# wzx99/DCFP

Hardware: AMD Instinct MI355X
Metric: training images/sec at 1024x2048 DeepLabv3-R101 (higher is better)
Workload: dtype f32; 1 GPU; DeepLabv3-resnet101+ASPP os8, 4x3x1024x2048 per GPU, CE+0.4*deepsup CE (fused upsample), 3x3 stride-1 convs with >= 256 channels as fp32 Winograd F(2x2,3x3) (fwd / dgrad / wgrad), all other convs direct implicit GEMM, EIC step, SGD m0.9 wd5e-4; global_batch=4, parallelism=dp1

## Files before the change

dcfp_amd/_lib.py:

```python
import ctypes as C
import os
import subprocess
import threading

_HERE = os.path.dirname(os.path.abspath(__file__))
LIB_PATH = os.environ.get("DCFP_LIB") or os.path.join(_HERE, "libdcfp_hip.so")
CSRC = os.path.join(_HERE, "csrc")

_lib = None
_lock = threading.Lock()


class ConvDesc(C.Structure):
    _fields_ = [(n, C.c_int32) for n in
                ("N", "Cin", "H", "W", "Cout", "KH", "KW", "stride", "pad", "dil", "Hout", "Wout",
                 "x_pitch", "dy_pitch")]


class ConvF16Desc(C.Structure):
    _fields_ = [(n, C.c_int32) for n in
                ("N", "H", "W", "Cin8", "x_pitch", "Cout", "K", "stride", "pad", "dil", "Hout", "Wout",
                 "y_pitch", "y_off", "res_pitch", "res_off", "relu")]


# ... 43 lines not shown

class VoteMap(C.Structure):
    _fields_ = [("logits", C.c_void_p)] + [(n, C.c_int32) for n in ("h", "w", "hs", "ws", "flip")] + \
               [("weight", C.c_float)]


AUG_SATURATION, AUG_HUE = 1, 2
SGD_CHUNK = 16384
CONV_FWD, CONV_DGRAD, CONV_WGRAD = 0, 1, 2
E_BADDESC, E_UNSUPPORTED, E_WORKSPACE = -1, -2, -3

_P, _I, _L, _F, _Z = C.c_void_p, C.c_int, C.c_int64, C.c_float, C.c_size_t
_D = C.POINTER(ConvDesc)
_R = C.POINTER(BnRunning)
_H = C.POINTER(ConvF16Desc)

SIGNATURES = {
    "dcfp_abi_version": (_I, []),
    "dcfp_conv2d_workspace_bytes": (_Z, [_D, _I]),
    "dcfp_conv2d_wp_layout": (_I, [_D, _I, C.POINTER(WpEntry)]),
    "dcfp_conv2d_permute_weights_multi_f32": (_I, [_P, _I, _L, _P]),
    "dcfp_conv2d_pitch_supported": (_I, [_D]),
    "dcfp_conv2d_kernel_name": (_I, [_D, _I, C.c_char_p, _I]),
    "dcfp_conv2d_executed_fraction": (C.c_double, [_D, _I]),
    "dcfp_conv2d_workspace_is_scratch": (_I, [_D, _I]),
    "dcfp_conv2d_dgrad_fanin_supported": (_I, [_D]),
    "dcfp_conv2d_dgrad_fanin_f32_nchw": (_I, [_D, _P, _L, _P, _P, _P, _P, _P, _Z, _I, _P]),
    "dcfp_conv2d_dgrad_fanin_red_slots": (_L, [_D]),
    "dcfp_conv2d_dgrad_fanin_red_f32_nchw": (_I, [_D, _P, _L, _P, _P, _P, _P, _P, _P, _P, _P, _P, _Z, _I, _P]),
    "dcfp_bn_bwd_sums_from_partials_f32": (_I, [_P, _L, _I, _P, _F, _P, _P, _P, _P, _P]),
    "dcfp_conv2d_xform_bytes": (_Z, [_D]),
    "dcfp_conv2d_fwd_keep_f32_nchw": (_I, [_D, _P, _P, _P, _L, _P, _Z, _P, _P, _Z, _P]),
    "dcfp_conv2d_wgrad_kept_f32_nchw": (_I, [_D, _P, _L, _P, _Z, _P, _P, _Z, _P]),
    "dcfp_conv2d_fwd_f32_nchw": (_I, [_D, _P, _P, _P, _P, _L, _P, _Z, _I, _P]),
    "dcfp_conv2d_fwd_fused_f32_nchw": (_I, [_D, _P, _P, _P, _P, _P, _I, _P, _P, _Z, _I, _P]),
    "dcfp_conv2d_dgrad_f32_nchw": (_I, [_D, _P, _L, _P, _P, _I, _P, _Z, _I, _P]),
    "dcfp_conv2d_wgrad_f32_nchw": (_I, [_D, _P, _L, _P, _P, _P, _P, _Z, _P]),
    "dcfp_bn_workspace_bytes": (_Z, [_I, _I, _I]),
    "dcfp_bn_stats_f32": (_I, [_P, _L, _I, _I, _I, _P, _P, _R, _P, _Z, _P]),
    "dcfp_bn_apply_f32": (_I, [_P, _P, _P, _P, _P, _F, _P, _I, _P, _L, _I, _I, _I, _I, _I, _P]),
    "dcfp_bn_bwd_reduce_f32": (_I, [_P, _L, _P, _P, _L, _P, _P, _P, _P, _F, _I, _I, _I, _I, _P, _P, _P, _P,
                                    _P, _Z, _P]),
    "dcfp_bn_update_running_f32": (_I, [_P, _P, _I, _F, _F, _P, _P, _P, _P]),
    "dcfp_syncbn_combine_f32": (_I, [_P, _I, _I, _P, _P, _P, _R, _P]),
    "dcfp_syncbn_p2p_mailbox_bytes": (_Z, [_I, _I]),
    "dcfp_p2p_alloc": (_I, [_Z, _I, C.POINTER(C.c_void_p)]),
    "dcfp_p2p_free": (_I, [_P]),
    "dcfp_p2p_export": (_I, [_P, _P]),
    "dcfp_p2p_import": (_I, [_P, C.POINTER(C.c_void_p)]),
    "dcfp_p2p_unmap": (_I, [_P]),
    "dcfp_syncbn_p2p_exchange_f32": (_I, [C.POINTER(C.c_void_p), _I, _I, C.c_uint32, _I, _P, _I, _I, _P, _R,
                                          C.c_uint32, _P, _P]),
    "dcfp_bn_apply_relu_mask_f32": (_I, [_P, _P, _P, _P, _P, _F, _P, _P, _P, _I, _I, _I, _P]),
    "dcfp_conv2d_fwd_stat_slots": (_L, [_D, _P, _L]),
    "dcfp_conv2d_fwd_stats_f32_nchw": (_I, [_D, _P, _P, _P, _L, _P, _P, _Z, _I, _P]),
    "dcfp_bn_stats_from_partials_f32": (_I, [_P, _L, _I, _I, _P, _P, _R, _P]),
    "dcfp_bn_bwd_apply_f32": (_I, [_P, _L, _P, _P, _L, _P, _P, _P, _P, _F, _P, _P, _F, _P, _I, _P, _P,
                                   _I, _I, _I, _I, _I, _P]),
    "dcfp_bn_bwd_fused_sync_bytes": (_Z, [_I, _I, _I]),
    "dcfp_bn_bwd_fused_f32": (_I, [_P, _L, _P, _P, _L, _P, _P, _P, _P, _F, _F, _I, _P, _P, _I, _I, _I, _I, _I,
                                   _P, _P, _P, _P, _P, _Z, C.c_uint32, C.c_uint32, _P, _P]),
    "dcfp_maxpool3x3s2_fwd_f32": (_I, [_P, _P, _P, _I, _I, _I, _I, _I, _I, _P]),
    "dcfp_maxpool3x3s2_bwd_f32": (_I, [_P, _P, _P, _I, _I, _I, _I, _I, _I, _P]),
    "dcfp_rowsum_f32": (_I, [_P, _L, _P, _F, _I, _I, _I, _P]),
    "dcfp_broadcast_hw_f32": (_I, [_P, _F, _P, _L, _I, _I, _I, _I, _P]),
    "dcfp_add_f32": (_I, [_P, _P, _P, _L, _P]),
# ... 89 lines not shown
```

dcfp_amd/csrc/conv_igemm2.hip:

```cpp
#include "igemm2_common.h"
#include <queue>
#include <vector>
#include <stdio.h>
#include <stdlib.h>

namespace {

__device__ __forceinline__ int wp_row(int m, int perm8) {
    if (!perm8) return m;
    const int j = m & 255;
    return (m & ~255) + 32 * (j & 7) + (j >> 3);
}

__global__ void __launch_bounds__(256)
permute_weights_kernel(const float* __restrict__ w, float* __restrict__ wp, int T, int Ck, int CkP,
                       int M, int Mpad, int sAm, int sAc, int perm8) {
    const long long total = (long long)T * CkP * Mpad;
    for (long long i = (long long)blockIdx.x * 256 + threadIdx.x; i < total;
         i += (long long)gridDim.x * 256) {
        const int m = wp_row((int)(i % Mpad), perm8);
        const long long r = i / Mpad;
        const int c = (int)(r % CkP);
        const int t = (int)(r / CkP);
        float v = 0.f;
        if (m < M && c < Ck) v = w[(long long)m * sAm + (long long)c * sAc + t];
        wp[i] = v;
    }
}

constexpr int kWpBlockElems = DCFP_WP_BLOCK_ELEMS;
__global__ void __launch_bounds__(256)
permute_weights_multi_kernel(const DcfpWpEntry* __restrict__ table, int n) {
    const long long blk = blockIdx.x;
    int lo = 0, hi = n - 1;
    while (lo < hi) {
        const int mid = (lo + hi + 1) >> 1;
        if (table[mid].first_block <= blk) lo = mid; else hi = mid - 1;
    }
    const DcfpWpEntry e = table[lo];
    const long long base = (blk - e.first_block) * kWpBlockElems;
    if (e.perm8 >= 2) {
        const long long pairs = (long long)e.CkP * e.Mpad;
#pragma unroll 1
        for (int u = 0; u < kWpBlockElems / 256; ++u) {
            const long long i = base + u * 256 + threadIdx.x;
            if (i >= pairs) return;
            wino_filter2_pair(e.w, e.sAm, e.sAc, e.perm8 == 3, e.M, e.Ck, e.Mpad, i, e.wp);
        }
        return;
    }
    const long long total = (long long)e.T * e.CkP * e.Mpad;
#pragma unroll
    for (int u = 0; u < kWpBlockElems / 256; ++u) {
        const long long i = base + u * 256 + threadIdx.x;
        if (i >= total) return;
        const int m = wp_row((int)(i % e.Mpad), e.perm8);
        const long long r = i / e.Mpad;
        const int c = (int)(r % e.CkP);
        const int t = (int)(r / e.CkP);
        float v = 0.f;
        if (m < e.M && c < e.Ck) v = e.w[(long long)m * e.sAm + (long long)c * e.sAc + t];
        e.wp[i] = v;
    }
}

__device__ __forceinline__ float half_xor(float v, int mask) {
    switch (mask) {
        case 1: return __builtin_bit_cast(float, __builtin_amdgcn_ds_swizzle(__builtin_bit_cast(int, v), (1 << 10) | 0x1f));
        case 2: return __builtin_bit_cast(float, __builtin_amdgcn_ds_swizzle(__builtin_bit_cast(int, v), (2 << 10) | 0x1f));
        case 4: return __builtin_bit_cast(float, __builtin_amdgcn_ds_swizzle(__builtin_bit_cast(int, v), (4 << 10) | 0x1f));
        case 8: return __builtin_bit_cast(float, __builtin_amdgcn_ds_swizzle(__builtin_bit_cast(int, v), (8 << 10) | 0x1f));
        default: return __builtin_bit_cast(float, __builtin_amdgcn_ds_swizzle(__builtin_bit_cast(int, v), (16 << 10) | 0x1f));
    }
}

template <int TAPS, int TM, int TN, int WM, int WN, bool SD, bool ACC, int KB = 16>
__global__ void __launch_bounds__(64 * WM * WN, (TM * TN <= 8 && WM * WN == 4 && !ACC) ? 2 : 1)
igemm2_kernel(const Igemm2Params p) {
    constexpr int BK = KB;
    constexpr int NPART = BK / 4;
    constexpr int BM = WM * TM * 32, BN = WN * TN * 32, NT = 64 * WM * WN;
    constexpr int AX = BM / 4;
    constexpr int AROWS = (NT / AX) < BK ? (NT / AX) : BK;
    constexpr int APASS = BK / AROWS;
    constexpr int TX = BN / 4, TY = NT / TX, RPT = BK / TY;
    static_assert(APASS >= 1 && APASS * AROWS == BK, "A loader shape");
    static_assert(TY >= 1 && RPT >= 1 && TY * RPT == BK, "B loader shape");

    extern __shared__ __attribute__((aligned(16))) float smem[];
    float* As = smem;
    float* Bs = smem + 2 * BK * BM;

    const int group = 8 * p.tiles_m;
    const int g = blockIdx.x / group, local = blockIdx.x - g * group;
    const int nt = g * 8 + (local & 7);
// ... 880 lines not shown
    }
    return mode;
}

double dcfp_igemm2_exec_fraction(int T, int M, int Ck, int N, int Hi, int Wi, int Ho, int Wo, int sn, int sd,
                                 int off0, int offstep, bool pitched) {
    if (T != 9 || sn != 1 || sd != 1) return 1.0;
    const long long px = (long long)N * Ho * Wo;
    const bool d8 = dcfp_igemm2_use_dma8(T, M, Ho * Wo, px, sn, sd, off0, offstep, Hi * Wi, Wo, pitched);
    if (!d8 && !dcfp_igemm2_dma_shape(T, M, Ck, Ho * Wo, px, sn, sd, off0, Hi * Wi, Wo)) return 1.0;
    Igemm2Params p = {};
    p.N = N; p.Hi = Hi; p.Wi = Wi; p.Ho = Ho; p.Wo = Wo; p.P = Ho * Wo; p.off0 = off0; p.offstep = offstep;
    p.tiles_per_img = (p.P + 255) / 256; p.tiles_n_total = p.tiles_per_img * N; p.tiles_m = (M + 255) / 256;
    {
        static const int t2d = [] { const char* e = getenv("DCFP_IGEMM_2D"); return e ? atoi(e) : 5; }();
        const bool fits = (t2d == 4 || t2d == 5) && Hi % (256 >> t2d) == 0 && Wi % (1 << t2d) == 0;
        p.tile2d = (!d8 && fits && !pitched && ((off0 | offstep) & 3) != 0 && Ho == Hi && Wo == Wi) ? t2d : 0;
    }
    if (pick_tapskip(p, 256) == 0) return 1.0;
    long long live = 0;
    for (int ti = 0; ti < p.tiles_per_img; ++ti) live += tile_live_rows(p, ti);
    return (double)live / (3.0 * p.tiles_per_img);
}

void dcfp_igemm2_wp_layout(int T, int M, int Ck, int P, long long px, int sn, int sd, int off0, int offstep, int HiWi,
                           int Wo, bool pitched, int sAm, int sAc, DcfpWpEntry* e) {
    const TileCfg c = pick_cfg(M, px, sd);
    const bool d8 = dcfp_igemm2_use_dma8(T, M, P, px, sn, sd, off0, offstep, HiWi, Wo, pitched);
    e->T = T; e->Ck = Ck; e->CkP = round_up(Ck, ck_pad()); e->M = M; e->Mpad = round_up(M, d8 ? 256 : c.bm);
    e->sAm = sAm; e->sAc = sAc; e->perm8 = d8 ? 1 : 0;
}

int dcfp_igemm2_permute_multi(const DcfpWpEntry* table, int n, long long total_blocks, hipStream_t stream) {
    hipLaunchKernelGGL(permute_weights_multi_kernel, dim3((unsigned)total_blocks), dim3(256), 0, stream, table, n);
    DCFP_RETURN_LAUNCH();
}

bool dcfp_igemm2_persist() {
    static const bool persist = [] { const char* e = getenv("DCFP_IGEMM_PERSIST"); return !e || atoi(e) != 0; }();
    return persist;
}

bool dcfp_igemm2_dma_shape(int T, int M, int Ck, int P, long long px, int sn, int sd, int off0, int HiWi, int Wo) {
    static const bool dma = [] { const char* e = getenv("DCFP_IGEMM_DMA"); return !e || atoi(e) != 0; }();
    static const bool dma9 = [] { const char* e = getenv("DCFP_IGEMM_DMA9"); return !e || atoi(e) != 0; }();
    if (!dma || pick_cfg(M, px, sd).id != 4 || sn != 1 || sd != 1 || HiWi != P || Wo % 4 != 0) return false;
    return T == 1 ? off0 == 0 : dma9;
}

int dcfp_igemm2_run(const float* in, long long in_nstride, const float* w, int sAm, int sAc,
                    const float* bias, float* out, long long out_nstride, int N, int M, int Ck, int T,
                    int Hi, int Wi, int Ho, int Wo, int sn, int sd, int off0, int offstep,
                    int accumulate, void* workspace, size_t workspace_bytes, hipStream_t stream,
                    const float* scale, const float* shift, const float* residual, int relu,
                    float* stat_part, int wp_valid, int in_pitch, long long wp_nstride, const float* fan_src,
                    const unsigned long long* fan_mask, const Igemm2Red* red) {
    const long long px = (long long)N * Ho * Wo;
    const TileCfg c = pick_cfg(M, px, sd);
    Igemm2Params p;
    p.stat_part = stat_part;
    p.wp_nstride = wp_nstride;
    p.fan_src = fan_src; p.fan_mask = fan_mask;
    p.red_x = red ? red->x : nullptr; p.red_mask = red ? red->mask : nullptr;
    p.red_mean = red ? red->mean : nullptr; p.red_part = red ? red->part : nullptr;
    if (red && !fan_src) return DCFP_E_BADDESC;
    p.in = in; p.bias = bias; p.out = out;
    p.scale = scale; p.shift = shift; p.residual = residual; p.relu = relu;
// ... 88 lines not shown
```

dcfp_amd/csrc/conv_winograd3.hip:

```cpp
#include "wino_patch.h"
#include <stdlib.h>

namespace {

constexpr int GBK = 8;
constexpr int GKH = 144;
constexpr int GHALF = 2 * GKH;
constexpr int GCOMP = 2 * GHALF;
constexpr int GSTAGE = 16 * GCOMP;
constexpr unsigned kSat = 0xffffffffu;

struct WinoWgParams {
    const float* x_base;
    unsigned x_bytes;
    const float* dy_base;
    unsigned dy_bytes;
    const unsigned* table;
    unsigned table_bytes;
    float* out;
    int M, C, mblocks, cblocks, nblk;
    unsigned x_chan_bytes, dy_chan_bytes;
    int kchunk;
    long long T16;
    int d;
};

__global__ void __launch_bounds__(256) wino_wg_table_kernel(unsigned* __restrict__ table, long long npairs, long long T, int N,
                                                            int H, int W, int d, int TH, int TW, long long x_nstride,
                                                            int x_pitch, int lead, long long dy_nstride, int dy_pitch, int dm) {
    const long long pi = (long long)blockIdx.x * 256 + threadIdx.x;
    if (pi >= npairs) return;
    unsigned e[8] = {kOob, kOob, kOob, kOob, kOob, kOob, 0u, 0u};
    const long long t = 2 * pi;
    if (t < T) {
// ... 326 lines not shown
    if (d >= 4 && d % 2 == 0 && W % 2 == 0) return 4;
    return -1;
}

WgPlan wg_plan(int N, int H, int W, int d, int M, int C) {
    WgPlan pl;
    pl.TH = d * ((H + 2 * d - 1) / (2 * d));
    pl.TW = d * ((W + 2 * d - 1) / (2 * d));
    pl.TW = (pl.TW + 3) / 4 * 4;
    pl.T = (long long)N * pl.TH * pl.TW;
    pl.T16 = (pl.T + 15) / 16 * 16;
    pl.mblocks = (M + 63) / 64;
    pl.cblocks = (C + 63) / 64;
    const long long tiles = (long long)pl.mblocks * pl.cblocks, slots = dcfp_num_cus();
    long long max_splits = pl.T16 / (32 * GBK);
    if (max_splits < 1) max_splits = 1;
    long long splits = 1;
    double best = -1.0;
    for (long long sp = 1; sp <= max_splits && tiles * sp <= 2 * slots; ++sp) {
        const long long blocks = tiles * sp, rounds = (blocks + slots - 1) / slots;
        const double eff = (double)blocks / (double)(rounds * slots);
        if (eff > best + 0.02) { best = eff; splits = sp; }
    }
    long long kchunk = (pl.T16 + splits - 1) / splits;
    kchunk = (kchunk + 15) / 16 * 16;
    splits = (pl.T16 + kchunk - 1) / kchunk;
    pl.splits = (int)splits;
    pl.kchunk = (int)kchunk;
    pl.table_floats = (pl.T16 / 2 * 8 + 63) / 64 * 64;
    pl.slab_floats = (long long)pl.splits * 16 * M * C;
    return pl;
}

}

bool dcfp_wino_wgrad_fused_enabled() {
    static const int v = [] { const char* e = getenv("DCFP_WINO_WGRAD_FUSED"); return e ? atoi(e) : 1; }();
    return v != 0;
}

bool dcfp_wino_wgrad_fused_ok(int N, int H, int W, int d, int M, int C, long long x_nstride, int x_pitch,
                              long long dy_nstride, int dy_pitch) {
    if (!dcfp_wino_wgrad_fused_enabled()) return false;
    if (M < 48 || C < 48) return false;
    if (x_pitch <= 0) x_pitch = W;
    if (dy_pitch <= 0) dy_pitch = W;
    if (wg_mode(N, H, W, d, M, C, x_nstride, x_pitch, dy_nstride, dy_pitch) < 0) return false;
    const WgPlan pl = wg_plan(N, H, W, d, M, C);
    if (pl.T16 >= (1LL << 30) || pl.T16 / 2 * 32 >= 0x7fffff00LL) return false;
    if (16LL * M * C * 4 >= 0x7fffff00LL) return false;
    return (long long)pl.mblocks * pl.cblocks * pl.splits < (1LL << 28);
}

size_t dcfp_wino_wgrad_fused_workspace_bytes(int N, int H, int W, int d, int M, int C) {
    const WgPlan pl = wg_plan(N, H, W, d, M, C);
    return (size_t)(pl.table_floats + pl.slab_floats) * sizeof(float);
}

int dcfp_wino_wgrad_fused_run(const float* dy, long long dy_nstride, int dy_pitch, const float* x, long long x_nstride,
                              int x_pitch, float* dw, int N, int M, int C, int H, int W, int d, void* workspace,
                              size_t workspace_bytes, hipStream_t stream) {
    if (x_pitch <= 0) x_pitch = W;
    if (dy_pitch <= 0) dy_pitch = W;
    const int mode = wg_mode(N, H, W, d, M, C, x_nstride, x_pitch, dy_nstride, dy_pitch);
    if (mode < 0) return DCFP_E_UNSUPPORTED;
    const WgPlan pl = wg_plan(N, H, W, d, M, C);
    if (!workspace || !dcfp_aligned16(workspace) || workspace_bytes < dcfp_wino_wgrad_fused_workspace_bytes(N, H, W, d, M, C))
        return DCFP_E_WORKSPACE;
    unsigned* table = static_cast<unsigned*>(workspace);
    float* slabs = static_cast<float*>(workspace) + pl.table_floats;
    const int lead = mode == 4 ? 0 : 4;
    const long long npairs = pl.T16 / 2;
    hipLaunchKernelGGL(wino_wg_table_kernel, dim3((unsigned)((npairs + 255) / 256)), dim3(256), 0, stream, table, npairs, pl.T,
                       N, H, W, d, pl.TH, pl.TW, x_nstride, x_pitch, lead, dy_nstride, dy_pitch, mode);
    WinoWgParams p;
    p.x_base = x - lead;
    p.x_bytes = (unsigned)(((long long)(N - 1) * x_nstride + (long long)C * H * x_pitch + lead) * 4);
    p.dy_base = dy;
    p.dy_bytes = (unsigned)(((long long)(N - 1) * dy_nstride + (long long)M * H * dy_pitch) * 4);
    p.table = table;
    p.table_bytes = (unsigned)(npairs * 32);
    p.out = slabs;
    p.M = M; p.C = C; p.mblocks = pl.mblocks; p.cblocks = pl.cblocks;
    p.nblk = pl.mblocks * pl.cblocks * pl.splits;
    p.x_chan_bytes = (unsigned)((long long)H * x_pitch * 4);
    p.dy_chan_bytes = (unsigned)((long long)H * dy_pitch * 4);
    p.kchunk = pl.kchunk;
    p.T16 = pl.T16;
    p.d = d;
    const unsigned grid = (unsigned)(((p.nblk + 7) / 8) * 8);
    const size_t lds = (size_t)4 * GSTAGE * sizeof(float);
    auto launch = [&](auto kern) -> int {
        hipError_t e = hipFuncSetAttribute(reinterpret_cast<const void*>(kern), hipFuncAttributeMaxDynamicSharedMemorySize,
                                           (int)lds);
        if (e != hipSuccess) return (int)e;
        hipLaunchKernelGGL(kern, dim3(grid), dim3(256), lds, stream, p);
        hipError_t e2 = hipGetLastError();
        return e2 == hipSuccess ? DCFP_OK : (int)e2;
    };
    const bool ragged = (M % 64) != 0 || (C % 64) != 0;
    int rc;
#define DCFP_WG(DM_) (ragged ? launch(wino_wgrad_fused_kernel<DM_, true>) : launch(wino_wgrad_fused_kernel<DM_, false>))
    switch (mode) {
        case 1: rc = DCFP_WG(1); break;
        case 2: rc = DCFP_WG(2); break;
        default: rc = DCFP_WG(4); break;
    }
// ... 7 lines not shown
```

dcfp_amd/ops.py:

```python
import ctypes as C
import os
import weakref

import torch
import torch.distributed as dist

from . import _lib, arena, syncbn_p2p
from ._lib import ConvDesc, BnRunning, check

_ws_cache = {}
WEIGHT_EPOCH = [0]

_PROFILE = None


def profile_start():
    global _PROFILE
    _PROFILE = []


def profile_stop():
    global _PROFILE
    recs, _PROFILE = _PROFILE, None
    torch.cuda.synchronize()
# ... 406 lines not shown
        raise RuntimeError("conv2d_wgrad: dw must be a contiguous tensor of the weight shape")
    if need_bias and db is None:
        db = torch.empty((wshape[0],), dtype=torch.float32, device=x.device)
    if xform is not None and not need_bias and L.dcfp_conv2d_xform_bytes(C.byref(d)) == xform.numel():
        _timed("conv_wgrad", d, _conv_flops(d), lambda: check(
            L.dcfp_conv2d_wgrad_kept_f32_nchw(C.byref(d), _p(dy), ns, _p(xform), xform.numel(), _p(dw), _p(ws), ws.numel(),
                                              _stream()), "conv2d_wgrad_kept"))
        return dw, None
    _timed("conv_wgrad", d, _conv_flops(d), lambda: check(
        L.dcfp_conv2d_wgrad_f32_nchw(C.byref(d), _p(dy), ns, _p(x), _p(dw), _p(db) if need_bias else None, _p(ws),
                                     ws.numel(), _stream()), "conv2d_wgrad"))
    return dw, (db if need_bias else None)


def add_into(dst, src):
    check(_lib.lib().dcfp_add_f32(_p(dst), _p(src), _p(dst), dst.numel(), _stream()), "add")


def wgrad_into_param(dy, x, w, bias, stride, pad, dil, keep=None):
    tw, kw = arena.grad_target(w)
    tb, kb = arena.grad_target(bias) if bias is not None else (None, 0)
    xform = keep.pop("xform", None) if keep else None
    conv2d_wgrad(dy, x, tuple(w.shape), stride, pad, dil, need_bias=bias is not None, dw=tw, db=tb, xform=xform)
    dw = arena.grad_commit(w, tw, kw, add_into)
    db = arena.grad_commit(bias, tb, kb, add_into) if bias is not None else None
    return dw, db


class Conv2dFn(torch.autograd.Function):

    @staticmethod
    def forward(ctx, x, w, bias, stride, pad, dil):
        ctx.keep = {} if ctx.needs_input_grad[1] else None
        y = conv2d_fwd(x, w, bias, stride, pad, dil, keep=ctx.keep)
        ctx.save_for_backward(x)
        ctx.params = (w, bias)
        ctx.cfg = (stride, pad, dil)
        return y

    @staticmethod
    def backward(ctx, dy):
        (x,) = ctx.saved_tensors
        w, bias = ctx.params
        stride, pad, dil = ctx.cfg
        dx = dw = db = None
        if ctx.needs_input_grad[0]:
            dx = conv2d_dgrad(dy, w, tuple(x.shape), stride, pad, dil)
        if ctx.needs_input_grad[1] or (bias is not None and ctx.needs_input_grad[2]):
            dw, db = wgrad_into_param(dy, x, w, bias, stride, pad, dil, keep=ctx.keep)
        return dx, dw, db, None, None, None


def conv2d(x, w, bias=None, stride=1, pad=0, dil=1):
    return Conv2dFn.apply(x, w, bias, stride, pad, dil)


def bn_stats(x, run=None):
    _require(x, "x")
    N, Cc, H, W = x.shape
    x, ns = _batch_strided(x)
    L = _lib.lib()
    ws = _workspace("bn", L.dcfp_bn_workspace_bytes(N, Cc, H * W), x.device)
    mean = torch.empty(Cc, dtype=torch.float32, device=x.device)
    var = torch.empty(Cc, dtype=torch.float32, device=x.device)
    _timed("bn_stats", None, 4.0 * x.numel(), lambda: check(
        L.dcfp_bn_stats_f32(_p(x), ns, N, Cc, H * W, _p(mean), _p(var), _rp(run), _p(ws), ws.numel(), _stream()),
        "bn_stats"))
    return mean, var


def bn_apply(x, mean, var, gamma, beta, eps, residual=None, relu=False, out=None):
    N, Cc, H, W = x.shape
    x = x.contiguous()
    if residual is not None:
        residual = residual.contiguous()
    yns, ypitch = 0, 0
    if out is None:
        y = torch.empty_like(x)
    else:
        y = out
# ... 809 lines not shown
        levels, widths, offs, fshape, align, training, eps = ctx.cfg
        nst = len(widths)
        saved = ctx.saved_tensors
        pooled, cs, flat = saved[:nst], saved[nst:2 * nst], saved[2 * nst:]
        tensors = ctx.params
        N, Cf, H, W = fshape
        need_dx = ctx.needs_input_grad[0]
        grads = [None] * (3 * nst)
        dys = ppm_resize_adjoint(dcat[:, :offs[nst]], widths, levels, align)
        dp = torch.empty(sum(N * Cf * a * b for a, b in levels), dtype=torch.float32, device=dcat.device) \
            if need_dx else None
        dps = _level_views(dp, N, [Cf] * nst, levels) if need_dx else None
        pending = None
        for k in range(nst):
            w, g, b = tensors[3 * k:3 * k + 3]
            res = bn_backward_impl(dys[k], cs[k], None, g, b, _bn_state(ctx.meta, flat, k), True, training[k], eps[k], False,
                                   between=pending)
            d_c, grads[3 * k + 1], grads[3 * k + 2] = res[0], res[1], res[2]
            if pending is not None:
                grads[3 * (k - 1)] = res[4]
            if need_dx:
                conv2d_dgrad(d_c, w, tuple(pooled[k].shape), 1, 0, 1, out=dps[k])
            pending = (lambda d_c=d_c, w=w, x=pooled[k]: wgrad_into_param(d_c, x, w, None, 1, 0, 1)[0])
        grads[3 * (nst - 1)] = pending()
        dfeats = ppm_pool_adjoint(dp, levels, fshape, g=dcat[:, offs[nst]:]) if need_dx else None
        _release_pitch(ctx)
        return (dfeats, None) + tuple(grads)


def pyramid_pooling(feats, cfg, tensors):
    return PyramidPoolingFn.apply(feats, cfg, *tensors)


class ForkFn(torch.autograd.Function):

    @staticmethod
    def forward(ctx, x):
        ctx.set_materialize_grads(False)
        return x.view_as(x), x.view_as(x)

    @staticmethod
    def backward(ctx, ga, gb):
        if ga is None or gb is None:
            return ga if gb is None else gb
        return add(ga, gb)


def fork(x):
    return ForkFn.apply(x) if (torch.is_grad_enabled() and x.requires_grad) else (x, x)


class MaxPool3x3s2Fn(torch.autograd.Function):

    @staticmethod
    def forward(ctx, x):
        _require(x, "x")
        x = x.contiguous()
        N, Cc, H, W = x.shape
        Ho, Wo = (H + 2 - 3) // 2 + 1, (W + 2 - 3) // 2 + 1
        y = torch.empty((N, Cc, Ho, Wo), dtype=torch.float32, device=x.device)
        idx = torch.empty((N, Cc, Ho, Wo), dtype=torch.int32, device=x.device)
        check(_lib.lib().dcfp_maxpool3x3s2_fwd_f32(_p(x), _p(y), _p(idx), N, Cc, H, W, Ho, Wo, _stream()),
              "maxpool_fwd")
        ctx.save_for_backward(idx)
        ctx.shape = (N, Cc, H, W, Ho, Wo)
        return y

    @staticmethod
    def backward(ctx, dy):
        (idx,) = ctx.saved_tensors
        N, Cc, H, W, Ho, Wo = ctx.shape
        dy = dy.contiguous()
        dx = torch.empty((N, Cc, H, W), dtype=torch.float32, device=dy.device)
        check(_lib.lib().dcfp_maxpool3x3s2_bwd_f32(_p(dy), _p(idx), _p(dx), N, Cc, H, W, Ho, Wo, _stream()),
              "maxpool_bwd")
        return dx


def maxpool3x3s2(x):
    return MaxPool3x3s2Fn.apply(x)


# ... 495 lines not shown
```

include/dcfp_hip.h:

```cpp
#ifndef DCFP_HIP_H
#define DCFP_HIP_H

#include <stddef.h>
#include <stdint.h>

#ifdef __cplusplus
extern "C" {
#endif

#define DCFP_OK 0
#define DCFP_E_BADDESC (-1)
#define DCFP_E_UNSUPPORTED (-2)
#define DCFP_E_WORKSPACE (-3)

typedef void* dcfp_stream_t;

int dcfp_abi_version(void);

typedef struct DcfpConvDesc {
    int32_t N, Cin, H, W;
    int32_t Cout, KH, KW;
    int32_t stride, pad, dil;
    int32_t Hout, Wout;
    int32_t x_pitch, dy_pitch;
} DcfpConvDesc;

enum { DCFP_CONV_FWD = 0, DCFP_CONV_DGRAD = 1, DCFP_CONV_WGRAD = 2 };

size_t dcfp_conv2d_workspace_bytes(const DcfpConvDesc* d, int pass);

#define DCFP_WP_BLOCK_ELEMS 2048
typedef struct DcfpWpEntry {
    const float* w;
    float* wp;
    int64_t first_block;
    int64_t n_blocks;
    int32_t T, Ck, CkP, M, Mpad, sAm, sAc;
    int32_t perm8;
} DcfpWpEntry;
int dcfp_conv2d_wp_layout(const DcfpConvDesc* d, int pass, DcfpWpEntry* entry);
int dcfp_conv2d_permute_weights_multi_f32(const DcfpWpEntry* table, int n_entries, int64_t total_blocks,
                                          dcfp_stream_t stream);

int dcfp_conv2d_pitch_supported(const DcfpConvDesc* d);

int dcfp_conv2d_workspace_is_scratch(const DcfpConvDesc* d, int pass);

size_t dcfp_conv2d_xform_bytes(const DcfpConvDesc* d);
int dcfp_conv2d_fwd_keep_f32_nchw(const DcfpConvDesc* d, const float* x, const float* w, float* y, int64_t y_nstride,
                                  float* xform_out, size_t xform_bytes,
                                  float* stat_partials ,
                                  void* workspace, size_t workspace_bytes, dcfp_stream_t stream);
int dcfp_conv2d_wgrad_kept_f32_nchw(const DcfpConvDesc* d, const float* dy, int64_t dy_nstride, const float* xform,
                                    size_t xform_bytes, float* dw, void* workspace, size_t workspace_bytes,
                                    dcfp_stream_t stream);

int dcfp_conv2d_dgrad_fanin_supported(const DcfpConvDesc* d);
int dcfp_conv2d_dgrad_fanin_f32_nchw(const DcfpConvDesc* d, const float* dy, int64_t dy_nstride, const float* w, float* dx,
                                     const float* fan_src, const void* fan_mask, void* workspace, size_t workspace_bytes,
                                     int wp_valid, dcfp_stream_t stream);
int64_t dcfp_conv2d_dgrad_fanin_red_slots(const DcfpConvDesc* d);
int dcfp_conv2d_dgrad_fanin_red_f32_nchw(const DcfpConvDesc* d, const float* dy, int64_t dy_nstride, const float* w,
                                         float* dx, const float* fan_src, const void* fan_mask, const float* red_x,
                                         const void* red_mask, const float* red_mean, float* red_part, void* workspace,
                                         size_t workspace_bytes, int wp_valid, dcfp_stream_t stream);
int dcfp_bn_bwd_sums_from_partials_f32(const float* partials, int64_t slots, int C, const float* var, float eps,
                                       float* sum_dy, float* sum_dy_xmu, float* dgamma ,
                                       float* dbeta , dcfp_stream_t stream);

int dcfp_conv2d_kernel_name(const DcfpConvDesc* d, int pass, char* buf, int buf_len);

double dcfp_conv2d_executed_fraction(const DcfpConvDesc* d, int pass);

int dcfp_conv2d_fwd_f32_nchw(const DcfpConvDesc* d, const float* x, const float* w,
                             const float* bias, float* y, int64_t y_nstride,
                             void* workspace, size_t workspace_bytes, int wp_valid,
                             dcfp_stream_t stream);
int dcfp_conv2d_fwd_fused_f32_nchw(const DcfpConvDesc* d, const float* x, const float* w,
                                   const float* scale, const float* shift, const float* residual,
                                   int relu, float* y, void* workspace, size_t workspace_bytes,
                                   int wp_valid, dcfp_stream_t stream);
int dcfp_conv2d_dgrad_f32_nchw(const DcfpConvDesc* d, const float* dy, int64_t dy_nstride,
                               const float* w, float* dx, int accumulate,
                               void* workspace, size_t workspace_bytes, int wp_valid,
                               dcfp_stream_t stream);
int dcfp_conv2d_wgrad_f32_nchw(const DcfpConvDesc* d, const float* dy, int64_t dy_nstride,
                               const float* x, float* dw, float* db,
                               void* workspace, size_t workspace_bytes,
// ... 282 lines not shown
```

Before: 12.16 images/s.

## Tile weight permutation via LDS, cache Winograd wgrad tables, fuse fork dgrad accumulation

Adds a tiled weight-permutation kernel that stages weights through shared memory so that global reads and writes are coalesced, with a Winograd filter-transform path built the same way. It also caches the Winograd wgrad index table per shape in a persistent device buffer, so the table kernel is not relaunched on every call. Separately, it defers the dgrad of a conv that consumes a fork tap so the result can be accumulated straight into the trunk gradient, avoiding a separate add. These changes add persistent allocations, global cache state and more complex autograd bookkeeping that depends on graph-task ids.

Result: no change. 12.16 images/s, median of 2 (+0.1%).

```diff
diff --git a/dcfp_amd/_lib.py b/dcfp_amd/_lib.py
--- a/dcfp_amd/_lib.py
+++ b/dcfp_amd/_lib.py
@@ -99,6 +99,7 @@
     "dcfp_conv2d_xform_bytes": (_Z, [_D]),
     "dcfp_conv2d_fwd_keep_f32_nchw": (_I, [_D, _P, _P, _P, _L, _P, _Z, _P, _P, _Z, _P]),
     "dcfp_conv2d_wgrad_kept_f32_nchw": (_I, [_D, _P, _L, _P, _Z, _P, _P, _Z, _P]),
+    "dcfp_wino_wgrad_table_launches": (_L, []),
     "dcfp_conv2d_fwd_f32_nchw": (_I, [_D, _P, _P, _P, _P, _L, _P, _Z, _I, _P]),
     "dcfp_conv2d_fwd_fused_f32_nchw": (_I, [_D, _P, _P, _P, _P, _P, _I, _P, _P, _Z, _I, _P]),
     "dcfp_conv2d_dgrad_f32_nchw": (_I, [_D, _P, _L, _P, _P, _I, _P, _Z, _I, _P]),
diff --git a/dcfp_amd/csrc/conv_igemm2.hip b/dcfp_amd/csrc/conv_igemm2.hip
--- a/dcfp_amd/csrc/conv_igemm2.hip
+++ b/dcfp_amd/csrc/conv_igemm2.hip
@@ -29,16 +29,17 @@
 }
 
 constexpr int kWpBlockElems = DCFP_WP_BLOCK_ELEMS;
-__global__ void __launch_bounds__(256)
-permute_weights_multi_kernel(const DcfpWpEntry* __restrict__ table, int n) {
-    const long long blk = blockIdx.x;
+__device__ __forceinline__ DcfpWpEntry wp_entry_of_block(const DcfpWpEntry* __restrict__ table, int n, long long blk) {
     int lo = 0, hi = n - 1;
     while (lo < hi) {
         const int mid = (lo + hi + 1) >> 1;
         if (table[mid].first_block <= blk) lo = mid; else hi = mid - 1;
     }
-    const DcfpWpEntry e = table[lo];
-    const long long base = (blk - e.first_block) * kWpBlockElems;
+    return table[lo];
+}
+
+__device__ __forceinline__ void wp_block_elements(const DcfpWpEntry& e, long long lb) {
+    const long long base = lb * kWpBlockElems;
     if (e.perm8 >= 2) {
         const long long pairs = (long long)e.CkP * e.Mpad;
 #pragma unroll 1
@@ -61,6 +62,175 @@
         float v = 0.f;
         if (m < e.M && c < e.Ck) v = e.w[(long long)m * e.sAm + (long long)c * e.sAc + t];
         e.wp[i] = v;
+    }
+}
+
+__global__ void __launch_bounds__(256)
+permute_weights_multi_kernel(const DcfpWpEntry* __restrict__ table, int n) {
+    const DcfpWpEntry e = wp_entry_of_block(table, n, blockIdx.x);
+    wp_block_elements(e, (long long)blockIdx.x - e.first_block);
+}
+
+constexpr int kWpRowsMax = 144;
+constexpr int kWpRowsMax8 = 36;
+constexpr int kWinoGPitch = 64 * 9 + 1;
+constexpr int kWpLdsFloats = 8 * kWinoGPitch + 16 * 512;
+
+typedef const float __attribute__((address_space(1)))* wp_src_t;
+typedef float __attribute__((address_space(1)))* wp_dst_t;
+constexpr int kWpBatch = 12;
+
+template <int TT, int MTT, int NCT, bool BYROW>
+__device__ __forceinline__ void wp_tile_permute(const DcfpWpEntry& e, long long tile, int MTr, int NCr, float* s) {
+    const int tid = threadIdx.x;
+    const int T = TT ? TT : e.T, MT = TT ? MTT : MTr, NC = TT ? NCT : NCr;
+    const int pitch = MT + 1;
+    const int mtiles = (e.Mpad + MT - 1) / MT;
+    const int ct = (int)(tile / mtiles), mt = (int)(tile - (long long)ct * mtiles);
+    const int m0 = mt * MT, c0 = ct * NC;
+    const int total = MT * NC * T;
+    const int run = (BYROW ? NC : MT) * T;
+    const wp_src_t w = (wp_src_t)e.w;
+    const wp_dst_t wp = (wp_dst_t)e.wp;
+    const int perm8 = e.perm8;
+    for (int base = 0; base < total; base += 256 * kWpBatch) {
+        float v[kWpBatch];
+        int at[kWpBatch];
+#pragma unroll
+        for (int u = 0; u < kWpBatch; ++u) {
+            const int i = base + u * 256 + tid;
+            const int o = i / run, r = i - o * run;
+            const int q = r / T, t = r - q * T;
+            const int ml = BYROW ? o : q, cl = BYROW ? q : o;
+            const int pos = perm8 ? 8 * (ml & 31) + (ml >> 5) : ml;
+            const int m = m0 + ml, c = c0 + cl;
+            at[u] = i < total ? (cl * T + t) * pitch + pos : -1;
+            v[u] = 0.f;
+            if (i < total && m < e.M && c < e.Ck) v[u] = w[(long long)m * e.sAm + (long long)c * e.sAc + t];
+        }
+#pragma unroll
+        for (int u = 0; u < kWpBatch; ++u)
+            if (at[u] >= 0) s[at[u]] = v[u];
+    }
+    __syncthreads();
+    const int quads = MT / 4, lines = NC * T;
+    for (int i = tid; i < lines * quads; i += 256) {
+        const int line = i / quads, q = i - line * quads;
+        const int t = line / NC, cl = line - t * NC;
+        const int c = c0 + cl, mq = m0 + 4 * q;
+        if (c >= e.CkP || mq >= e.Mpad) continue;
+        const float* src = s + (cl * T + t) * pitch + 4 * q;
+        const f32x4 v = {src[0], src[1], src[2], src[3]};
+        *reinterpret_cast<f32x4 __attribute__((address_space(1)))*>(wp + ((long long)t * e.CkP + c) * e.Mpad + mq) = v;
+    }
+    __syncthreads();
+}
+
+template <bool BYROW>
+__device__ __forceinline__ void wp_tile_wino(const DcfpWpEntry& e, long long tile, float* s) {
+    const int tid = threadIdx.x;
+    const int mblocks = e.Mpad / 64;
+    const int cb = (int)(tile / mblocks), mb = (int)(tile - (long long)cb * mblocks);
+    const int m0 = 64 * mb, c0 = 8 * cb;
+    float* gs = s;
+    float* us = s + 8 * kWinoGPitch;
+    constexpr int run = (BYROW ? 8 : 64) * 9;
+    const wp_src_t w = (wp_src_t)e.w;
+    float v[18];
+    int at[18];
+#pragma unroll
+    for (int u = 0; u < 18; ++u) {
+        const int i = u * 256 + tid;
+        const int o = i / run, r = i - o * run;
+        const int q = r / 9, t = r - q * 9;
+        const int ml = BYROW ? o : q, cl = BYROW ? q : o;
+        const int m = m0 + ml, c = c0 + cl;
+        at[u] = cl * kWinoGPitch + 9 * ml + t;
+        v[u] = 0.f;
+        if (m < e.M && c < e.Ck) v[u] = w[(long long)m * e.sAm + (long long)c * e.sAc + t];
+    }
+#pragma unroll
+    for (int u = 0; u < 18; ++u) gs[at[u]] = v[u];
+    __syncthreads();
+    const bool flip = e.perm8 == 3;
+#pragma unroll
+    for (int h = 0; h < 2; ++h) {
+        const int kk = tid & 3, lane = tid >> 2;
+        const int cl = 2 * kk + (lane >> 5), ml = 32 * h + (lane & 31);
+        const float* src = gs + cl * kWinoGPitch + 9 * ml;
+        float g[9];
+#pragma unroll
+        for (int t = 0; t < 9; ++t) g[t] = src[flip ? 8 - t : t];
+        float r[4][3];
+#pragma unroll
+        for (int k = 0; k < 3; ++k) {
+            const float g0 = g[k], g1 = g[3 + k], g2 = g[6 + k];
+            r[0][k] = g0;
+            r[1][k] = 0.5f * ((g0 + g2) + g1);
+            r[2][k] = 0.5f * ((g0 + g2) - g1);
+            r[3][k] = g2;
+        }
+        float* dst = us + 256 * h + tid;
+#pragma unroll
+        for (int i = 0; i < 4; ++i) {
+            const float a = r[i][0], b = r[i][1], cc = r[i][2];
+            dst[(4 * i + 0) * 512] = a;
+            dst[(4 * i + 1) * 512] = 0.5f * ((a + cc) + b);
+            dst[(4 * i + 2) * 512] = 0.5f * ((a + cc) - b);
+            dst[(4 * i + 3) * 512] = cc;
+        }
+    }
+    __syncthreads();
+    f32x4 __attribute__((address_space(1)))* out =
+        reinterpret_cast<f32x4 __attribute__((address_space(1)))*>((wp_dst_t)e.wp + tile * (16 * 512));
+    const f32x4* us4 = reinterpret_cast<const f32x4*>(us);
+#pragma unroll
+    for (int u = 0; u < 8; ++u) out[u * 256 + tid] = us4[u * 256 + tid];
+    __syncthreads();
+}
+
+__device__ __forceinline__ bool wp_entry_tiled_ok(const DcfpWpEntry& e) {
+    if (e.n_blocks <= 0 || (reinterpret_cast<uintptr_t>(e.wp) & 15u)) return false;
+    if (e.perm8 >= 2) return e.CkP % 8 == 0 && e.Mpad % 64 == 0;
+    if (e.perm8 == 1 && e.Mpad % 256 != 0) return false;
+    return e.Mpad % 4 == 0 && e.T >= 1 && e.T <= (e.perm8 ? kWpRowsMax8 : kWpRowsMax);
+}
+
+__global__ void __launch_bounds__(256)
+permute_weights_multi_tiled_kernel(const DcfpWpEntry* __restrict__ table, int n) {
+    __shared__ __attribute__((aligned(16))) float s[kWpLdsFloats];
+    const DcfpWpEntry e = wp_entry_of_block(table, n, blockIdx.x);
+    const long long lb = (long long)blockIdx.x - e.first_block;
+    if (!wp_entry_tiled_ok(e)) {
+        wp_block_elements(e, lb);
+        return;
+    }
+    const bool by_row = e.sAm > e.sAc;
+    if (e.perm8 >= 2) {
+        const long long tiles = (long long)(e.CkP / 8) * (e.Mpad / 64);
+        for (long long tile = lb; tile < tiles; tile += e.n_blocks) {
+            if (by_row) wp_tile_wino<true>(e, tile, s);
+            else wp_tile_wino<false>(e, tile, s);
+        }
+        return;
+    }
+    const int MT = e.perm8 ? 256 : 64;
+    const int rows = e.perm8 ? kWpRowsMax8 : kWpRowsMax;
+    int NC = rows / e.T;
+    if (NC > (e.perm8 ? 32 : 64)) NC = e.perm8 ? 32 : 64;
+    const long long tiles = (long long)((e.Mpad + MT - 1) / MT) * ((e.CkP + NC - 1) / NC);
+    const int kind = (e.T == 1 ? 0 : e.T == 9 ? 2 : 4) + (e.perm8 ? 1 : 0);
+    for (long long tile = lb; tile < tiles; tile += e.n_blocks) {
+#define DCFP_WP_TILE(T_, MT_, NC_) \
+    (by_row ? wp_tile_permute<T_, MT_, NC_, true>(e, tile, MT, NC, s) : wp_tile_permute<T_, MT_, NC_, false>(e, tile, MT, NC, s))
+        switch (kind) {
+            case 0: DCFP_WP_TILE(1, 64, 64); break;
+            case 1: DCFP_WP_TILE(1, 256, 32); break;
+            case 2: DCFP_WP_TILE(9, 64, 16); break;
+            case 3: DCFP_WP_TILE(9, 256, 4); break;
+            default: DCFP_WP_TILE(0, 0, 0); break;
+        }
+#undef DCFP_WP_TILE
     }
 }
 
@@ -1007,7 +1177,11 @@
 }
 
 int dcfp_igemm2_permute_multi(const DcfpWpEntry* table, int n, long long total_blocks, hipStream_t stream) {
-    hipLaunchKernelGGL(permute_weights_multi_kernel, dim3((unsigned)total_blocks), dim3(256), 0, stream, table, n);
+    static const bool tiled = [] { const char* e = getenv("DCFP_WP_REFRESH_TILED"); return !e || atoi(e) != 0; }();
+    if (tiled)
+        hipLaunchKernelGGL(permute_weights_multi_tiled_kernel, dim3((unsigned)total_blocks), dim3(256), 0, stream, table, n);
+    else
+        hipLaunchKernelGGL(permute_weights_multi_kernel, dim3((unsigned)total_blocks), dim3(256), 0, stream, table, n);
     DCFP_RETURN_LAUNCH();
 }
 
diff --git a/dcfp_amd/csrc/conv_winograd3.hip b/dcfp_amd/csrc/conv_winograd3.hip
--- a/dcfp_amd/csrc/conv_winograd3.hip
+++ b/dcfp_amd/csrc/conv_winograd3.hip
@@ -1,5 +1,9 @@
 #include "wino_patch.h"
 #include <stdlib.h>
+#include <atomic>
+#include <map>
+#include <mutex>
+#include <tuple>
 
 namespace {
 
@@ -392,7 +396,80 @@
     return pl;
 }
 
-}
+struct WgTableKey {
+    int dev, N, H, W, d, mode, x_pitch, dy_pitch;
+    long long x_nstride, dy_nstride;
+    bool operator<(const WgTableKey& o) const {
+        return std::tie(dev, N, H, W, d, mode, x_pitch, dy_pitch, x_nstride, dy_nstride) <
+               std::tie(o.dev, o.N, o.H, o.W, o.d, o.mode, o.x_pitch, o.dy_pitch, o.x_nstride, o.dy_nstride);
+    }
+};
+
+std::atomic<long long> g_wg_table_launches{0};
+
+void wg_table_launch(unsigned* table, const WgTableKey& k, const WgPlan& pl, int lead, hipStream_t stream) {
+    const long long npairs = pl.T16 / 2;
+    hipLaunchKernelGGL(wino_wg_table_kernel, dim3((unsigned)((npairs + 255) / 256)), dim3(256), 0, stream, table, npairs, pl.T,
+                       k.N, k.H, k.W, k.d, pl.TH, pl.TW, k.x_nstride, k.x_pitch, lead, k.dy_nstride, k.dy_pitch, k.mode);
+    g_wg_table_launches.fetch_add(1, std::memory_order_relaxed);
+}
+
+bool wg_table_cached() {
+    static const bool on = [] { const char* e = getenv("DCFP_WINO_WG_TABLE_CACHE"); return !e || atoi(e) != 0; }();
+    return on;
+}
+
+struct WgTableEntry {
+    unsigned* table;
+    hipStream_t stream;
+    hipEvent_t built;
+    bool done;
+};
+
+const unsigned* wg_cached_table(WgTableKey key, const WgPlan& pl, int lead, hipStream_t stream) {
+    static std::mutex mu;
+    static std::map<WgTableKey, WgTableEntry> cache;
+    if (hipGetDevice(&key.dev) != hipSuccess) return nullptr;
+    std::lock_guard<std::mutex> lock(mu);
+    auto it = cache.find(key);
+    if (it == cache.end()) {
+        WgTableEntry e = {nullptr, stream, nullptr, false};
+        if (hipMalloc(reinterpret_cast<void**>(&e.table), (size_t)pl.table_floats * sizeof(float)) != hipSuccess) {
+            (void)hipGetLastError();
+            return nullptr;
+        }
+        if (hipEventCreateWithFlags(&e.built, hipEventDisableTiming) != hipSuccess) {
+            (void)hipGetLastError();
+            (void)hipFree(e.table);
+            return nullptr;
+        }
+        wg_table_launch(e.table, key, pl, lead, stream);
+        if (hipEventRecord(e.built, stream) != hipSuccess) {
+            (void)hipGetLastError();
+            (void)hipStreamSynchronize(stream);
+            e.done = true;
+        }
+        it = cache.emplace(key, e).first;
+        return it->second.table;
+    }
+    WgTableEntry& e = it->second;
+    if (!e.done && stream != e.stream) {
+        if (hipEventQuery(e.built) == hipSuccess) {
+            e.done = true;
+        } else {
+            (void)hipGetLastError();
+            if (hipStreamWaitEvent(stream, e.built, 0) != hipSuccess) {
+                (void)hipGetLastError();
+                return nullptr;
+            }
+        }
+    }
+    return e.table;
+}
+
+}
+
+extern "C" int64_t dcfp_wino_wgrad_table_launches(void) { return g_wg_table_launches.load(std::memory_order_relaxed); }
 
 bool dcfp_wino_wgrad_fused_enabled() {
     static const int v = [] { const char* e = getenv("DCFP_WINO_WGRAD_FUSED"); return e ? atoi(e) : 1; }();
@@ -427,12 +504,16 @@
     const WgPlan pl = wg_plan(N, H, W, d, M, C);
     if (!workspace || !dcfp_aligned16(workspace) || workspace_bytes < dcfp_wino_wgrad_fused_workspace_bytes(N, H, W, d, M, C))
         return DCFP_E_WORKSPACE;
-    unsigned* table = static_cast<unsigned*>(workspace);
     float* slabs = static_cast<float*>(workspace) + pl.table_floats;
     const int lead = mode == 4 ? 0 : 4;
     const long long npairs = pl.T16 / 2;
-    hipLaunchKernelGGL(wino_wg_table_kernel, dim3((unsigned)((npairs + 255) / 256)), dim3(256), 0, stream, table, npairs, pl.T,
-                       N, H, W, d, pl.TH, pl.TW, x_nstride, x_pitch, lead, dy_nstride, dy_pitch, mode);
+    const WgTableKey key = {0, N, H, W, d, mode, x_pitch, dy_pitch, x_nstride, dy_nstride};
+    const unsigned* table = wg_table_cached() ? wg_cached_table(key, pl, lead, stream) : nullptr;
+    if (!table) {
+        unsigned* own = static_cast<unsigned*>(workspace);
+        wg_table_launch(own, key, pl, lead, stream);
+        table = own;
+    }
     WinoWgParams p;
     p.x_base = x - lead;
     p.x_bytes = (unsigned)(((long long)(N - 1) * x_nstride + (long long)C * H * x_pitch + lead) * 4);
diff --git a/dcfp_amd/ops.py b/dcfp_amd/ops.py
--- a/dcfp_amd/ops.py
+++ b/dcfp_amd/ops.py
@@ -462,6 +462,7 @@
     @staticmethod
     def forward(ctx, x, w, bias, stride, pad, dil):
         ctx.keep = {} if ctx.needs_input_grad[1] else None
+        ctx.fork = getattr(x, "_dcfp_fork", None)
         y = conv2d_fwd(x, w, bias, stride, pad, dil, keep=ctx.keep)
         ctx.save_for_backward(x)
         ctx.params = (w, bias)
@@ -475,7 +476,12 @@
         stride, pad, dil = ctx.cfg
         dx = dw = db = None
         if ctx.needs_input_grad[0]:
-            dx = conv2d_dgrad(dy, w, tuple(x.shape), stride, pad, dil)
+            xshape = tuple(x.shape)
+
+            def dgrad(out=None):
+                return conv2d_dgrad(dy, w, xshape, stride, pad, dil, out=out, accumulate=out is not None)
+            if not _fork_defer(ctx.fork, dgrad):
+                dx = dgrad()
         if ctx.needs_input_grad[1] or (bias is not None and ctx.needs_input_grad[2]):
             dw, db = wgrad_into_param(dy, x, w, bias, stride, pad, dil, keep=ctx.keep)
         return dx, dw, db, None, None, None
@@ -1351,22 +1357,60 @@
     return PyramidPoolingFn.apply(feats, cfg, *tensors)
 
 
+FORK_ACCUMULATE = os.environ.get("DCFP_FORK_ACCUMULATE", "1") not in ("0",)
+
+
+def _graph_task():
+    f = getattr(torch._C, "_current_graph_task_id", None)
+    t = f() if f is not None else -1
+    return t if t >= 0 else None
+
+
+def _fork_defer(rec, dgrad):
+    task = _graph_task()
+    if rec is None or not FORK_ACCUMULATE or task is None:
+        return False
+    pending = rec.get("dgrad")
+    if pending is not None and pending[0] == task:
+        return False
+    tap = rec["tap"]()
+    if tap is None or tap._backward_hooks or tap.retains_grad:
+        return False
+    rec["dgrad"] = (task, dgrad)
+    return True
+
+
 class ForkFn(torch.autograd.Function):
 
     @staticmethod
-    def forward(ctx, x):
+    def forward(ctx, x, rec):
         ctx.set_materialize_grads(False)
+        ctx.rec = rec
         return x.view_as(x), x.view_as(x)
 
     @staticmethod
     def backward(ctx, ga, gb):
+        task, dgrad = ctx.rec.pop("dgrad", None) or (None, None)
+        if dgrad is not None and task == _graph_task():
+            trunk = ctx.rec["trunk"]()
+            watched = trunk is not None and (trunk._backward_hooks or trunk.retains_grad)
+            if ga is None and gb is not None and gb.is_contiguous() and gb.dtype == torch.float32 and not watched:
+                return dgrad(gb), None
+            v = dgrad()
+            ga = v if ga is None else add(v, ga)
         if ga is None or gb is None:
-            return ga if gb is None else gb
-        return add(ga, gb)
+            return (ga if gb is None else gb), None
+        return add(ga, gb), None
 
 
 def fork(x):
-    return ForkFn.apply(x) if (torch.is_grad_enabled() and x.requires_grad) else (x, x)
+    if not (torch.is_grad_enabled() and x.requires_grad):
+        return x, x
+    rec = {}
+    tap, trunk = ForkFn.apply(x, rec)
+    rec["tap"], rec["trunk"] = weakref.ref(tap), weakref.ref(trunk)
+    tap._dcfp_fork = rec
+    return tap, trunk
 
 
 class MaxPool3x3s2Fn(torch.autograd.Function):
diff --git a/include/dcfp_hip.h b/include/dcfp_hip.h
--- a/include/dcfp_hip.h
+++ b/include/dcfp_hip.h
@@ -54,6 +54,7 @@
 int dcfp_conv2d_wgrad_kept_f32_nchw(const DcfpConvDesc* d, const float* dy, int64_t dy_nstride, const float* xform,
                                     size_t xform_bytes, float* dw, void* workspace, size_t workspace_bytes,
                                     dcfp_stream_t stream);
+int64_t dcfp_wino_wgrad_table_launches(void);
 
 int dcfp_conv2d_dgrad_fanin_supported(const DcfpConvDesc* d);
 int dcfp_conv2d_dgrad_fanin_f32_nchw(const DcfpConvDesc* d, const float* dy, int64_t dy_nstride, const float* w, float* dx,
```
